# phonchi/Cryo-RAlib

Hardware: AMD Instinct MI355X
Metric: particles/sec aligned, 90x90 nref=10 xr=yr=3 ou=36 (higher is better)
Workload: dtype f32

## Files before the change

cryo_ralib_amd/api.py:

```python
import ctypes
import os

import numpy as np

from ._common import Launcher, ptr

_HERE = os.path.dirname(os.path.abspath(__file__))
LIB_PATH = os.environ.get("RALIGN_LIB") or os.path.join(_HERE, "libralign_hip.so")

RA_MODE_MREF = 0
RA_MODE_REFFREE = 1
RA_INTERP_BILINEAR = 0
RA_INTERP_QUADRI = 1


class AlignConfig(ctypes.Structure):
    _fields_ = [("sbj_num", ctypes.c_uint), ("ref_num", ctypes.c_uint), ("img_dim", ctypes.c_uint),
                ("ring_num", ctypes.c_uint), ("ring_len", ctypes.c_uint),
                ("shift_step", ctypes.c_float), ("shift_rng_x", ctypes.c_float), ("shift_rng_y", ctypes.c_float)]


class AlignParam(ctypes.Structure):
    _fields_ = [("sbj_id", ctypes.c_int), ("ref_id", ctypes.c_int), ("shift_x", ctypes.c_float),
                ("shift_y", ctypes.c_float), ("angle", ctypes.c_float), ("mirror", ctypes.c_bool)]
# ... 21 lines not shown


class RaLdsRow(ctypes.Structure):
    _fields_ = [("kernel", ctypes.c_char * 64), ("static_bytes", ctypes.c_int), ("dynamic_bytes", ctypes.c_int),
                ("limit_bytes", ctypes.c_int)]


float_ptr = ctypes.POINTER(ctypes.c_float)
aln_param_ptr = ctypes.POINTER(AlignParam)

EXPORTED_SYMBOLS = [
    "print_gpu_info", "gpu_clear", "pre_align_init", "pre_align_size_check", "pre_align_fetch",
    "pre_align_run", "pre_align_run_m", "mref_align_run", "mref_align_run_m", "get_num_ref", "reset_shifts",
    "ref_free_alignment_2D_init", "ref_free_alignment_2D_size_check", "ref_free_alignment_2D",
    "ref_free_alignment_2D_filter_references", "ra_isac_get_references", "ra_legacy_bytes",
    "ra_last_error", "ra_create", "ra_destroy", "ra_set_stream", "ra_num_shifts", "ra_maxrin", "ra_lcirc", "ra_search_path", "ra_search_tiled", "ra_search_offsets_per_pass", "ra_set_nomirror", "ra_set_mask",
    "ra_reset_shifts", "ra_set_references", "ra_get_prepared_references", "ra_align", "ra_state_from_params", "ra_set_refine", "ra_set_class_references", "ra_align_classes",
    "ra_debug_spectra", "ra_transform_accumulate", "ra_update_references", "ra_normalize_particles", "ra_sync", "ra_kernel_time",
    "ra_fsc_len", "ra_class_fsc", "ra_last_class_fsc", "ra_fit_tanh", "ra_class_averages", "ra_filter_references",
    "ra_state_from_params_dev", "ra_class_fsc_fit", "ra_filter_references_dev", "ra_last_refine_count", "ra_lds_report",
    "ra_create_ex", "ra_set_normalize_ring", "ra_get_options", "ra_search_skips_offsets", "ra_phase_flip",
    "ra_sdr_mean", "ra_sdr_gram", "ra_sdr_project", "ra_sdr_factors", "ra_rot_shift2d", "ra_sdr_reconstruct",
    "ra_tsne_knn", "ra_tsne_affinity", "ra_tsne_step", "ra_tsne_error",
    "ra_tsne_knn_query", "ra_tsne_affinity_rows", "ra_tsne_place_gradient", "ra_tsne_place",
    "ra_kmeans_sqnorm", "ra_kmeans_labels", "ra_kmeans_lloyd", "ra_kmeans_search", "ra_kmeans_seed",
    "ra_kmeans_silhouette", "ra_kmeans_dispersion", "ra_gmm_estep", "ra_gmm_mstep", "ra_dbscan_count", "ra_dbscan_step",
    "ra_hdbscan_core", "ra_hdbscan_round", "ra_ward_nearest", "ra_ward_merge", "ra_embed_ranks",
    "ra_spectral_spmv", "ra_spectral_lanczos", "ra_spectral_ritz", "ra_spectral_components", "ra_spectral_work_bytes",
    "ra_umap_smooth_knn", "ra_umap_epochs", "ra_umap_place",
    "ra_fourier_resize", "ra_wiener_accumulate", "ra_wiener_finalize", "ra_wiener_frc", "ra_wiener_finalize_ssnr", "ra_wiener_score",
    "ra_prep_normalize", "ra_prep_filter",
# ... 17 lines not shown
    L = ctypes.CDLL(p)
    vp = ctypes.c_void_p
    L.ra_last_error.restype = ctypes.c_char_p
    L.ra_create.argtypes = [ctypes.POINTER(vp), ctypes.POINTER(RaConfig)]
    L.ra_create_ex.argtypes = [ctypes.POINTER(vp), ctypes.POINTER(RaConfig), ctypes.POINTER(RaOptions)]
    L.ra_set_normalize_ring.argtypes = [vp, ctypes.c_int]
    L.ra_get_options.argtypes = [vp, ctypes.POINTER(RaOptions)]
    L.ra_destroy.argtypes = [vp]
    L.ra_destroy.restype = None
    L.ra_set_stream.argtypes = [vp, vp]
    L.ra_num_shifts.argtypes = [vp]
    L.ra_maxrin.argtypes = [vp]
    L.ra_lcirc.argtypes = [vp]
    L.ra_search_path.argtypes = [vp]
    L.ra_search_tiled.argtypes = [vp]
    L.ra_search_skips_offsets.argtypes = [vp]
    L.ra_search_offsets_per_pass.argtypes = [vp]
    L.ra_set_nomirror.argtypes = [vp, ctypes.c_int]
    L.ra_set_mask.argtypes = [vp, vp]
    L.ra_reset_shifts.argtypes = [vp, ctypes.c_float, ctypes.c_float, ctypes.c_float]
    L.ra_set_references.argtypes = [vp, vp]
    L.ra_get_prepared_references.argtypes = [vp, vp]
    L.ra_align.argtypes = [vp, vp, ctypes.c_int, vp, vp, float_ptr]
    L.ra_set_class_references.argtypes = [vp, vp, ctypes.c_int]
    L.ra_align_classes.argtypes = [vp, vp, ctypes.c_int, vp, vp, vp]
    L.ra_state_from_params.argtypes = [vp, vp, ctypes.c_int, float_ptr, vp]
    L.ra_set_refine.argtypes = [vp, ctypes.c_float]
    L.ra_last_refine_count.argtypes = [vp]
    L.ra_lds_report.argtypes = [vp, ctypes.POINTER(RaLdsRow), ctypes.c_int]
    L.ra_state_from_params_dev.argtypes = [vp, vp, ctypes.c_int, vp, vp]
# ... 497 lines not shown
    def align(self, particles, state, result, cs=None):
        n = particles.shape[0]
        assert particles.shape[1:] == (self.nx, self.nx) and state.shape == (n, 2) and result.shape == (n, 8)
        csp = None
        if cs is not None:
            csp = (ctypes.c_float * 2)(float(cs[0]), float(cs[1]))
        _check(self.lib.ra_align(self.handle, self._ptr(particles, self.torch.float32), n,
                                 self._ptr(state, self.torch.float32), self._ptr(result, self.torch.int32), csp),
               "ra_align")

    @property
    def search_tiled(self):
        return bool(self.lib.ra_search_tiled(self.handle))

    @property
    def search_skips_offsets(self):
        return bool(self.lib.ra_search_skips_offsets(self.handle))

    @property
    def search_offsets_per_pass(self):
        return self.lib.ra_search_offsets_per_pass(self.handle)

    def set_refine(self, threshold):
        _check(self.lib.ra_set_refine(self.handle, float(threshold)), "ra_set_refine")

    def state_from_params(self, result, state, cs=None):
        n = result.shape[0]
        assert state.shape == (n, 2) and result.shape == (n, 8)
        csp = None
        if cs is not None:
# ... 115 lines not shown
```

cryo_ralib_amd/csrc/ralign_engine.hip:

```cpp
#include <hip/hip_runtime.h>

#include <algorithm>
#include <cmath>
#include <cstdio>
#include <cstdlib>
#include <cstring>
#include <string>
#include <vector>

#include "ralign_geom.h"
#include "ralign_kernels.h"
#include "ralign_generic.h"
#include "ralign_xform.h"
#include "ralign_zone.h"
#include "ralign_fused.h"
#include "ralign_tiled.h"
#include "ralign_solo.h"
#include "ralign_duo.h"
#include "ralign_pair.h"
#include "ralign_exact.h"
#include "ralign_refine.h"
#include "ralign_host.h"
#include "ralign_plan.h"

// ... 228 lines not shown
    case 128: R1 = 16; R2 = 8; return true;
    case 256: R1 = 16; R2 = 16; return true;
    default: return false;
    }
}

typedef void (*gpolar_fn)(DevGeom, const float *, const float *, int, float *, float2 *);
static gpolar_fn gpolar_kernel(const ra_engine *e, bool refs)
{
    const bool q = e->dg.interp == RA_INTERP_QUADRI;
    return refs ? (q ? (gpolar_fn)polar_generic_kernel<true, true> : (gpolar_fn)polar_generic_kernel<true, false>)
                : (q ? (gpolar_fn)polar_generic_kernel<false, true> : (gpolar_fn)polar_generic_kernel<false, false>);
}

static fused_fn select_tiled(int nh, int sbuf);
static fused_fn select_fused(int maxrin, int nref, int nzr, int sbuf, bool pack = false, bool crop = false);
static bool tcrop_wanted(ra_engine *e, const PlanRequest &rq)
{
    const Geometry &g = e->geo;
    if (!tcrop_class(g, e->cfg, rq, e->generic)) return false;
    FusedGeom t{};
    crop_plan(g, t, rq.sw.crop);
    if (!t.s_crop) return false;
    const int sbuf = (g.lring + 31) / 32 * 32 + 16;
    FusedPlanHost tmp;
    const int pst_min = t.s_pst;
    for (int pst : {pst_min < 101 && !(RA_EXP_ENV("RALIGN_CROP_PST101") && ra_atoi(RA_EXP_ENV("RALIGN_CROP_PST101")) == 0) ? 101 : pst_min, pst_min}) {
    e->crop_pst = pst;
    const size_t polar = (size_t)pst * pst + 4 * (size_t)std::max(sbuf, sbuf <= RF_SBUF_FIXED ? RF_SBUF_FIXED : sbuf) + 2 * g.maxrin + 3000;
    const bool no_tiled = rq.sw.tiled == 0;
    for (int sb : {sbuf <= RF_SBUF_FIXED ? RF_SBUF_FIXED : sbuf, sbuf}) {
// ... 384 lines not shown
}

extern "C" const char *ra_last_error(void) { return g_last_error.c_str(); }

static ccf_fn select_ccf(int maxrin)
{
    switch (maxrin) {
    case 256: return ccf_kernel<256>;
    case 128: return ccf_kernel<128>;
    case 64: return ccf_kernel<64>;
    case 32: return ccf_kernel<32>;
    default: return nullptr;
    }
}

static fused_fn select_fused(int maxrin, int nref, int nzr, int sbuf, bool pack, bool crop)
{
    if (nref > RF_MAXREF) return nullptr;
    const int nrp = (nref + 1) / 2;
    const bool one = nzr == 1;
    if (crop) {
        if (maxrin != 256 || (pack && !one)) return nullptr;
        switch ((nrp + 1) / 2) {
        case 1: return pack ? search_fused_kernel<256, 1, true, 0, true, true> : one ? search_fused_kernel<256, 1, true, 0, false, true> : search_fused_kernel<256, 1, false, 0, false, true>;
        case 2: return pack ? search_fused_kernel<256, 2, true, 0, true, true> : one ? search_fused_kernel<256, 2, true, 0, false, true> : search_fused_kernel<256, 2, false, 0, false, true>;
        case 3: return pack ? search_fused_kernel<256, 3, true, 0, true, true> : one ? search_fused_kernel<256, 3, true, 0, false, true> : search_fused_kernel<256, 3, false, 0, false, true>;
        default: return pack ? search_fused_kernel<256, 4, true, 0, true, true> : one ? search_fused_kernel<256, 4, true, 0, false, true> : search_fused_kernel<256, 4, false, 0, false, true>;
        }
    }
    if (pack) {
        if (maxrin != 256 || !one) return nullptr;
        if (sbuf == RF_SBUF_FIXED)
            switch ((nrp + 1) / 2) {
            case 1: return search_fused_kernel<256, 1, true, RF_SBUF_FIXED, true>;
            case 2: return search_fused_kernel<256, 2, true, RF_SBUF_FIXED, true>;
// ... 84 lines not shown
    const bool no_tiled = rq.sw.tiled == 0;
    auto plan_tiled = [&]() { return build_tiled_plan(g, e->cfg.nref, e->dg.sbuf, e->lds_polar / sizeof(float), fp) && select_tiled(fp.f.nh, e->dg.sbuf); };
    auto plan_fused = [&]() { return select_fused(g.maxrin, e->cfg.nref, 1, 0, false, e->tcrop) && build_fused_plan(g, e->cfg.nref, e->dg.sbuf, e->lds_polar / sizeof(float), fp); };
    if (e->want.tiled && plan_tiled()) e->tiled = true;
    else if (plan_fused()) e->tiled = false;
    else if (e->tcrop && !no_tiled && plan_tiled()) e->tiled = true;
    else if (e->tcrop) {
        g_last_error = "particle-resident search over a crop: the plan tcrop_wanted promised does not fit";
        return RA_ERR_STATE;
    } else return RA_OK;
    if (e->tcrop) {
        FusedGeom tcr{};
        crop_plan(g, tcr, rq.sw.crop);
        fp.f.s_crop = tcr.s_crop; fp.f.s_cropm = tcr.s_cropm;
    }
    int rc;
    if ((rc = upload_resident_tables(e))) return rc;
    for (int pk = 0; pk < (e->tiled ? 1 : 2); pk++) {
        const fused_fn fk = e->tiled ? select_tiled(fp.f.nh, e->dg.sbuf) : select_fused(g.maxrin, e->cfg.nref, fp.f.nzr, e->dg.sbuf, pk != 0, e->tcrop);
        (pk ? e->search.pack : e->search.fused) = fk;
        if (!fk) continue;
        const std::string kn = std::string(e->tiled ? "search_tiled_kernel" : pk ? "search_fused_kernel<pack>" : "search_fused_kernel") + (e->tcrop ? " (crop)" : "");
        if ((rc = raise_dynamic_lds(e, (const void *)fk, kn.c_str(), fp.lds_bytes))) return rc;
    }
    e->search.lds = fp.lds_bytes;
    if (rq.sw.info) fprintf(stderr, "libralign_hip: %s plan: %zu bytes of LDS (polar part %zu), sbuf %d, pst %d, nzr %d, rz %d\n", e->tiled ? "tiled" : "fused", fp.lds_bytes, e->lds_polar, e->dg.sbuf, e->dg.pst, fp.f.nzr, fp.f.rz);
    e->fused = true;
    return RA_OK;
}

static solo_fn select_solo(int maxrin, int nh, int ntile)
{
    if (maxrin != 512) return nullptr;
    if (ntile > 1)
// ... 468 lines not shown
    if (hipStreamSynchronize(e->stream) != hipSuccess || hipMemcpy(&h, e->d_rcount, sizeof(int), hipMemcpyDeviceToHost) != hipSuccess) return RA_ERR_HIP;
    return h;
}
extern "C" int ra_lds_report(const ra_engine *e, ra_lds_row *rows, int cap)
{
    if (!e || cap < 0 || (cap > 0 && !rows)) return RA_ERR_ARG;
    const int n = (int)e->lds_rows.size();
    for (int i = 0; i < std::min(n, cap); i++) {
        const LdsRow &r = e->lds_rows[i];
        snprintf(rows[i].kernel, sizeof(rows[i].kernel), "%s", r.kernel.c_str());
        rows[i].static_bytes = r.stat; rows[i].dynamic_bytes = r.dyn; rows[i].limit_bytes = r.limit;
    }
    return n;
}
extern "C" int ra_search_tiled(const ra_engine *e) { return !e ? RA_ERR_ARG : (e->fused && e->tiled) ? 1 : 0; }
extern "C" int ra_search_path(const ra_engine *e) { return !e ? RA_ERR_ARG : e->solo ? 3 : e->fused ? 1 : e->generic ? 2 : 0; }
extern "C" int ra_search_offsets_per_pass(const ra_engine *e) { return !e ? RA_ERR_ARG : !e->solo ? 0 : (e->duo || e->pair) ? 2 : 1; }
extern "C" int ra_search_skips_offsets(const ra_engine *e) { return !e ? RA_ERR_ARG : (e->solo || e->dg.ent_base) ? 1 : 0; }
extern "C" int ra_num_shifts(const ra_engine *e) { return e ? e->geo.nshift : RA_ERR_ARG; }
extern "C" int ra_maxrin(const ra_engine *e) { return e ? e->geo.maxrin : RA_ERR_ARG; }
extern "C" int ra_lcirc(const ra_engine *e) { return e ? e->geo.lcirc : RA_ERR_ARG; }

extern "C" int ra_reset_shifts(ra_engine *e, float xrng, float yrng, float step)
{
    if (!e) return RA_ERR_ARG;
    const PlanRequest rq{read_switches(), e->force_generic, false, false};
    Geometry g2 = e->geo;
    if (!build_shifts(g2, xrng, yrng, step)) { g_last_error = "bad shift window"; return RA_ERR_ARG; }
    if (g2.nshift_pad > e->pad_cap || g2.nshift > e->shift_cap) {
        g_last_error = "reset_shifts: more search offsets than the engine was created with";
// ... 866 lines not shown
```

cryo_ralib_amd/csrc/ralign_fused.h:

```cpp
#pragma once

#include <algorithm>
#include <cstdlib>
#include <vector>

#include "ralign_geom.h"
#include "ralign_kernels.h"

namespace ralign {

constexpr int RF_WAVES = 16;
constexpr int RF_THREADS = RF_WAVES * 64;
constexpr int RF_MAXREF = 16;

struct FusedGeom {
    int on;
    int ng;
    int wpg;
    int nrp;
    int nrpw;
    int rz, nzr, rz_inv;
    int b_floats;
    int grp_ring0[16];
    int s_crop, s_cropm;
// ... 10 lines not shown
    int ntile, nh;
    int ifft_full;
    int s_pst, s_rows;
    int s_sbuf;
    int s_rank[16];
    int s_call[16];
    int s_stat, s_ctr, s_rec;
    int s_r2;
};

struct FusedPlanHost {
    FusedGeom f{};
    std::vector<int> bsrc;
    std::vector<float> cdc_w;
    size_t lds_bytes = 0;
};

inline int rf_bsrc_code(const Geometry &g, int k, int r, int ref, int part)
{
    if (r >= g.nring) return -1;
    const int n = g.numr[3 * r + 2];
    int ks = k;
    if (k == 0 && part == 1) {
        if (n != g.maxrin) return -1;
        ks = n / 2; part = 0;
    } else if (k > n / 2 || (k == n / 2 && n == g.maxrin)) return -1;
    else if (k == n / 2 && part == 1) return -1;
    const int e = g.bin_off[ks] + (r - g.bin_first[ks]);
    return (e << 8) | (ref << 1) | part;
}
// ... 242 lines not shown
    {
        if (!on) return;
#ifdef RALIGN_PROFILE_SWITCHES
        if (tl && threadIdx.x % 64 == 0) tl[13] = clock64();
#endif
        while (__builtin_amdgcn_readfirstlane(__hip_atomic_load(done, __ATOMIC_RELAXED, __HIP_MEMORY_SCOPE_WORKGROUP)) < target)
            __builtin_amdgcn_s_sleep(1);
        __builtin_amdgcn_fence(__ATOMIC_ACQUIRE, "workgroup", "local");
#ifdef RALIGN_PROFILE_SWITCHES
        if (tl && threadIdx.x % 64 == 0) tl[14] = clock64();
#endif
    }
};

#define RF_SBUF_FIXED 6432
template <int N, int NRPW, bool ONE, int SB, bool PACK = false, bool CROP = false>
__global__ __launch_bounds__(RF_THREADS) void search_fused_kernel(DevGeom g_in, FusedGeom f, const float *__restrict__ particles,
                                                                  const float *__restrict__ state, int n,
                                                                  const float *__restrict__ Bf0, int nref,
                                                                  CandT *__restrict__ cand, const int *__restrict__ cls)
{
    DevGeom g = g_in;
    g.maxrin = N; g.lg_maxrin = __builtin_ctz(N);
    if constexpr (SB != 0) g.sbuf = SB;
    constexpr int R1 = IfftPlan<N>::R1, R2 = IfftPlan<N>::R2;
    extern __shared__ __align__(16) float lds[];
    const int npad = g.pst * g.pst;
    float *img = lds;
    float *bufs = lds + ((npad + 3) & ~3);
    float2 *tw_s = reinterpret_cast<float2 *>(bufs + 4 * g.sbuf);
    float2 *qt_s = tw_s + g.maxrin;
    int4 *inst_s = reinterpret_cast<int4 *>(qt_s + g.n_qtab + (g.n_qtab & 1));
    int4 *jobs_s = inst_s + g.n_inst;
    float *instw_s = reinterpret_cast<float *>(jobs_s + g.n_job);
    float *red = instw_s + g.n_inst;
    float2 *tws = reinterpret_cast<float2 *>(red + 24 + 8 * g.nring + ((g.n_inst + 8 * g.nring) & 1));
// ... 59 lines not shown
            float *dst = img + (y + g.bd) * g.pst + g.bd;
#pragma unroll 1
            for (int c0 = 0; c0 < g.nx; c0 += 64)
                if (c0 + lane < g.nx)
                    __builtin_amdgcn_global_load_lds(row + c0 + lane, (__attribute__((address_space(3))) void *)(dst + c0), 4, 0, 0);
        }
        asm volatile("s_waitcnt vmcnt(0)" ::: "memory");
    };
    auto write_centre = [&](int i0, int s0, int k) {
        int i = i0, sk = s0 + k;
        if (sk >= SPP) { sk -= SPP; i++; }
        i = min(i, npw - 1);
        const int pk = particle_of(i);
        const Window wk = particle_window(g, state[2 * pk], state[2 * pk + 1]);
        const int si = min(sk, g.nshift - 1);
        red[16 + 2 * k] = ((float)g.cnx + wk.sxi) + g.shift_x[si];
        red[17 + 2 * k] = ((float)g.cnx + wk.syi) + g.shift_y[si];
        red[7] = 0.f;
    };
    if (tid < 4 && npw > 0) write_centre(0, 0, (int)tid);
    RF_LDS_BARRIER();
    const int4 jd0 = jobs_s[min((int)wave, g.n_job - 1)];
    constexpr bool defer = ONE;
    auto reduce_records = [&](int i0r, int s0r, int nl) {
        constexpr int W = sizeof(CandT) / 4;
        if (wave == 2 && lane < nl * W) {
            const int o = lane / W, wd = lane - o * W;
            float bv = pc[o * nref].val, sv = -3.0e38f; int br = 0, sr = 0;
            for (int q3 = 1; q3 < nref; q3++) {
                const float v = pc[o * nref + q3].val;
                if (v >= bv) { sv = bv; sr = br; bv = v; br = q3; }
                else if (v >= sv) { sv = v; sr = q3; }
// ... 16 lines not shown
        const int a = min(4, SPP - s0);
        const bool split = PACK && a < nlive;
        const float *Bf = cls ? Bf0 + (size_t)cls[particle_of(i0)] * f.b_floats : Bf0;
        const bool pend = defer && grp > 0;
        if (!RA_DBG(g, 16)) {
#pragma unroll 1
            for (int ph = 0; ph < (split ? 2 : 1); ph++) {
                if (img_i != i0 + ph) {
                    if (ph) RF_LDS_BARRIER();
                    load_image(i0 + ph);
                    img_i = i0 + ph;
                    RF_LDS_BARRIER();
                }
                const int slo = ph ? a : 0, shi = (split && !ph) ? a : nlive;
                const bool wait = pend && !ph;
#pragma unroll 1
                for (int jr = 0; jr * RF_WAVES < g.n_job; jr++) {
                    const int job = jr * RF_WAVES + wave;
                    if (job >= g.n_job) continue;
                    const int4 jd = jr == 0 ? jd0 : jobs_s[job];
#ifdef RALIGN_PROFILE_SWITCHES
                    const PassSync ps = {wait && jr == 0, ifft_done, done_target, g.timeline && tl && grp < 64 ? g.timeline + (grp * 16 + wave) * 16 : nullptr};
#else
                    const PassSync ps = {wait && jr == 0, ifft_done, done_target};
#endif
                    switch (__builtin_amdgcn_readfirstlane(jd.x)) {
                    case 1: ring_job<8, 8, true, true>(g, imgb, bufs, tw_s, qt_s, red + 16, red + 24, inst_s, instw_s, jd.y, jd.z, jd.w, g.sbuf, shi, ps, slo); break;
                    case 6: ring_job<16, 8, true, true>(g, imgb, bufs, tw_s, qt_s, red + 16, red + 24, inst_s, instw_s, jd.y, jd.z, jd.w, g.sbuf, shi, ps, slo); break;
                    case 7: ring_job<8, 4, true, true>(g, imgb, bufs, tw_s, qt_s, red + 16, red + 24, inst_s, instw_s, jd.y, jd.z, jd.w, g.sbuf, shi, ps, slo); break;
                    case 9: ring_job_mix<true>(g, imgb, bufs, tw_s, qt_s, red + 16, red + 24, inst_s, instw_s, jd.y, jd.z, jd.w, g.sbuf, shi, ps, slo); break;
                    default: break;
                    }
                }
                if (wait && wave >= g.n_job) { const PassSync ps = {true, ifft_done, done_target}; ps(); }
            }
        } else if (pend) {
            const PassSync ps = {true, ifft_done, done_target};
            ps();
        }
        if (pend) reduce_records(i0p, s0p, nlp);
        RA_STAMP(g, tl, grp, wave, 1);
        const int ln = __builtin_amdgcn_mbcnt_hi(~0u, __builtin_amdgcn_mbcnt_lo(~0u, __float_as_int(red[7])));
        float4 b0[NRPW];
        {
            const float *bp = Bf + f.grp_boff[xm] + ln * 4;
// ... 148 lines not shown
```

cryo_ralib_amd/csrc/ralign_kernels.h:

```cpp
#pragma once

#include <hip/hip_runtime.h>
#include <stdint.h>

#include "ralign_fft.h"
#include "../../include/ralign.h"

#ifdef RALIGN_PROFILE_SWITCHES
#define RA_DBG(g, bits) (((g).dbg & (bits)) != 0)
#define RA_STAMP(g, cond, grp, wave, s)                                                                         \
    do { if ((g).timeline && (cond) && (grp) < 64 && threadIdx.x % 64 == 0) (g).timeline[((grp) * 16 + (wave)) * 16 + (s)] = clock64(); } while (0)
#else
#define RA_DBG(g, bits) false
#define RA_STAMP(g, cond, grp, wave, s) do { } while (0)
#endif

namespace ralign {

typedef float f32x4 __attribute__((ext_vector_type(4)));

struct DevGeom {
    int nx, cnx;
    int nring, maxrin, lcirc, lring, nbins, LB, LBP;
    int last_ring;
// ... 137 lines not shown
    int idx;
    asm("v_mad_i32_i24 %0, %1, %2, %3" : "=v"(idx) : "v"(iy), "s"(st), "v"(ix));
    const float *p = base + idx;
#ifdef RALIGN_BILINEAR_EXACT_ORDER
    const float f00 = p[0], f10 = p[1], f01 = p[st], f11 = p[st + 1];
    return f00 + ydif * (f01 - f00) + xdif * (f10 - f00 + ydif * (f11 - f10 - f01 + f00));
#else
    const v2f r0 = {p[0], p[1]}, r1 = {p[st], p[st + 1]};
    const v2f g = __builtin_elementwise_fma((v2f){ydif, ydif}, r1 - r0, r0);
    float d = g.y - g.x;
    asm("" : "+v"(d));
    return __builtin_fmaf(xdif, d, g.x);
#endif
}

struct Window { float sxi, syi; int lkx, rkx, lky, rky; };
__device__ __forceinline__ Window particle_window(const DevGeom &g, float dx, float dy)
{
    Window w;
    const float mashi = (float)(g.cnx - g.win_ring - 2);
    if (g.mode == RA_MODE_MREF) {
        if (fabsf(dx) > mashi || fabsf(dy) > mashi) { dx = 0.f; dy = 0.f; }
    } else {
        dx = fminf(fmaxf(dx, -mashi), mashi);
        dy = fminf(fmaxf(dy, -mashi), mashi);
    }
    w.sxi = dx; w.syi = dy;
    const int cn = g.nx / 2 + 1;
    float qlx = fmaxf(cn + dx - g.win_ring - 2, 0.f), qex = fmaxf(g.nx - cn - dx - g.win_ring, 0.f);
    float qly = fmaxf(cn + dy - g.win_ring - 2, 0.f), qey = fmaxf(g.nx - cn - dy - g.win_ring, 0.f);
// ... 141 lines not shown
    do {                                                             \
        __builtin_amdgcn_fence(__ATOMIC_RELEASE, "workgroup");       \
        asm volatile("s_waitcnt lgkmcnt(0)" ::: "memory");           \
        __builtin_amdgcn_wave_barrier();                             \
        __builtin_amdgcn_fence(__ATOMIC_ACQUIRE, "workgroup");       \
    } while (0)

#ifdef RALIGN_MARK_PHASES
#define RA_PHASE_MARK(name) asm volatile("; RA_PHASE " name)
#else
#define RA_PHASE_MARK(name) do {} while (0)
#endif

struct NoSync { __device__ __forceinline__ void operator()() const {} };

template <int R1, int LR, bool NYQ1 = false, bool EARLY = false, class Sync = NoSync>
__device__ __forceinline__ void ring_job(const DevGeom &g, const float *imgb, float *bufs, const float2 *tw_s,
                                         const float2 *qt_s, const float *ctr, float *part, const int4 *inst_s,
                                         const float *instw_s, int inst0, int count, int zero, int sbuf, int nlive = 4,
                                         Sync sync = Sync(), int slot_lo = 0)
{
    const int lane = __builtin_amdgcn_mbcnt_hi(~0u, __builtin_amdgcn_mbcnt_lo(~0u, zero));

    constexpr int H = R1 * LR, NR = 2 * H, LT = NR / 4;
    const int sub = lane / LR, t = lane % LR;
    const int subc = min(sub, count - 1);
    const int4 in = inst_s[inst0 + subc];
    const int slot = in.x & 255, ring = in.x >> 8;
    const bool active = sub < count && slot < nlive && slot >= slot_lo;
    float *buf = bufs + (__mul24(slot, sbuf) + in.y);
    const float rad = (float)in.w, wt = instw_s[inst0 + subc];
    const float cx = ctr[2 * slot], cy = ctr[2 * slot + 1];
    const float2 *qt = qt_s + in.z;
    v2f av2 = {0.f, 0.f}, sq2 = {0.f, 0.f};
    const v2f ctr2 = {cx, cy};
    float2 v[R1];
    constexpr bool QCT = (2 * LR <= LT) && (R1 >= 4);
    constexpr int NB = QCT ? R1 / 4 : R1;
    auto table_index = [&](int step, int u, int &qd) {
        if constexpr (QCT) { qd = 0; return 2 * LR * step + 2 * t + u; }
        else { const int j = 2 * (LR * step + t) + u; qd = j / LT; return j % LT; }
    };
    if (active) {
    int qdn[2];
    float2 scn[2];
#pragma unroll
    for (int u = 0; u < 2; u++) scn[u] = qt[table_index(0, u, qdn[u])];
#pragma unroll
// ... 14 lines not shown
        for (int q = 0; q < (QCT ? 4 : 1); q++) {
            const int a = QCT ? q * NB + b : b;
            v2f val;
#pragma unroll
            for (int u = 0; u < 2; u++) {
                v2f o;
                if constexpr (QCT) {
                    o = q == 0 ? ctr2 + xy[u] : q == 1 ? vadd_rot<-1>(ctr2, xy[u]) : q == 2 ? ctr2 - xy[u] : vadd_rot<1>(ctr2, xy[u]);
                } else {
                    const int qd = qdc[u];
                    v2f m = (qd & 1) ? v2f{xy[u].y, xy[u].x} : xy[u];
                    m.x = (qd & 2) ? -m.x : m.x;
                    m.y = ((qd + 1) & 2) ? -m.y : m.y;
                    o = m + ctr2;
                }
                const float s = bilinear_pad(imgb, g.pst, o.x, o.y);
                if (u == 0) val.x = s; else val.y = s;
            }
            av2 += val;
            sq2 += val * val;
            v[a] = make_float2(val.x, val.y);
            if ((NYQ1 && (QCT ? 4 * b + q : b) >= R1 / 2) || ((QCT ? q : b) & 1)) __builtin_amdgcn_sched_barrier(0);
        }
    }
    }
    sync();
    if (!active) return;
    float av = (av2.x + av2.y) * wt, sq = (sq2.x + sq2.y) * wt;
    if (RA_DBG(g, 256)) {
#pragma unroll
        for (int a = 0; a < R1; a++) *reinterpret_cast<float2 *>(buf + 2 * (LR * a + t)) = v[a];
        return;
    }
    RA_PHASE_MARK("ring_fft_begin");
    Dft<-1, R1>::run(v);
    constexpr int LGH = __builtin_ctz(H), LGNR = LGH + 1;
    const int tstep = t << (g.lg_maxrin - LGH);
// ... 106 lines not shown
                } else {
                    float2 zm = *reinterpret_cast<const float2 *>(buf + 2 * (H - k));
                    v2f xk, xm;
                    vsplit_pair(to_v(zk), to_v(zm), to_v(tw_s[k << lsh]), xk, xm);
                    *reinterpret_cast<float2 *>(buf + 2 * k) = to_f2(xk);
                    if (2 * k != H) *reinterpret_cast<float2 *>(buf + 2 * (H - k)) = to_f2(xm);
                }
            }
        }
    }
    RA_PHASE_MARK("ring_fft_end");
    av = group_sum_dpp<LR>(av); sq = group_sum_dpp<LR>(sq);
    if (t == 0) { part[2 * (slot * g.nring + ring)] = av; part[2 * (slot * g.nring + ring) + 1] = sq; }
}

template <bool NYQ1, class Sync = NoSync>
__device__ __forceinline__ void ring_job_mix(const DevGeom &g, const float *imgb, float *bufs, const float2 *tw_s,
                                             const float2 *qt_s, const float *ctr, float *part, const int4 *inst_s,
                                             const float *instw_s, int inst0, int count, int zero, int sbuf, int nlive = 4,
                                             Sync sync = Sync(), int slot_lo = 0)
{
    const int lane = __builtin_amdgcn_mbcnt_hi(~0u, __builtin_amdgcn_mbcnt_lo(~0u, zero));
    const int lanec = min(lane, count - 1);
    const int4 in = inst_s[inst0 + lanec];
    const int slot = in.x & 255, ring = (in.x >> 8) & 255, lg = (in.x >> 16) & 15, t = in.x >> 20;
    const bool active = lane < count && slot < nlive && slot >= slot_lo;
    const int lgLR = lg - 3, LR = 1 << lgLR, H = 4 << lgLR, lgLT = lg - 2, LTm = (1 << lgLT) - 1;
    float *buf = bufs + (__mul24(slot, sbuf) + in.y);
    const float rad = (float)in.w, wt = instw_s[inst0 + lanec];
    const v2f ctr2 = {ctr[2 * slot], ctr[2 * slot + 1]};
    const float2 *qt = qt_s + in.z;
    v2f av2 = {0.f, 0.f}, sq2 = {0.f, 0.f};
    float2 v[4];
    if (active) {
#pragma unroll
    for (int a = 0; a < 4; a++) {
        v2f val;
#pragma unroll
        for (int u = 0; u < 2; u++) {
            const int j = 2 * ((a << lgLR) + t) + u, qd = j >> lgLT;
            const float2 sc = qt[j & LTm];
            v2f o;
            {
#pragma clang fp contract(off)
                const v2f xy = v2f{sc.x, sc.y} * rad;
                v2f m = (qd & 1) ? v2f{xy.y, xy.x} : xy;
                m.x = (qd & 2) ? -m.x : m.x;
                m.y = ((qd + 1) & 2) ? -m.y : m.y;
                o = m + ctr2;
            }
            const float sv = bilinear_pad(imgb, g.pst, o.x, o.y);
            if (u == 0) val.x = sv; else val.y = sv;
        }
        av2 += val;
        sq2 += val * val;
        v[a] = make_float2(val.x, val.y);
    }
    }
    sync();
    if (!active) return;
    Dft<-1, 4>::run(v);
    const int tstep = t << (g.lg_maxrin - (lg - 1));
#pragma unroll
    for (int c = 0; c < 4; c++) {
        float2 o = v[c];
        if (c > 0) o = cmul(o, tw_s[__mul24(tstep, c)]);
// ... 947 lines not shown
```

cryo_ralib_amd/csrc/ralign_plan.h:

```cpp
#pragma once

#include <cstdlib>

#include "../../include/ralign.h"
#include "ralign_geom.h"
#include "ralign_fused.h"
#include "ralign_tiled.h"
#include "ralign_solo.h"
#include "ralign_pair.h"

namespace ralign {

inline int env_int(const char *name, int unset) { const char *v = getenv(name); return v ? atoi(v) : unset; }
inline bool env_set(const char *name) { return getenv(name) != nullptr; }

struct PlanSwitches {
    bool generic, fused, solo, pair, duo, tcrop, crop, tight_rings, zones, live_offsets, gccf_split, refine_gm, atomic_sums, info;
    int tiled;
    int gccf_tm;
    int solo_jobs;
    int grid;
    const char *refine;
};
inline PlanSwitches read_switches()
// ... 48 lines not shown
}
inline bool duo_class(const Geometry &g, const ra_config &cfg, const PlanRequest &rq, bool generic)
{
    return solo_class(g, cfg, rq, generic) && rq.sw.duo;
}
inline bool pair_class(const Geometry &g, const ra_config &cfg, const PlanRequest &rq, bool generic)
{
    return generic && g.maxrin == 256 && g.nring <= 4 * RP_NQ && g.numr[2] >= 8 && cfg.nref <= 127 && !rq.generic_forced() && rq.sw.pair;
}
inline bool tcrop_class(const Geometry &g, const ra_config &cfg, const PlanRequest &rq, bool generic)
{
    return generic && g.maxrin == 256 && g.nring <= 64 && g.numr[2] >= 8 && cfg.nref <= 127 && !rq.generic_forced() &&
           rq.allow_tcrop && rq.sw.tcrop && rq.sw.fused;
}

inline size_t b_stream_quads(const Geometry &g)
{
    size_t quads = 0;
    for (int m = 0; m < g.maxrin / 32; m++) {
        int r0 = 0;
        while (r0 < g.nring) {
            const int n = g.numr[3 * r0 + 2], nbin = (n == g.maxrin) ? n / 2 : n / 2 + 1;
            if (16 * m < nbin) break;
            r0++;
        }
        quads += (g.nring - r0 + 3) / 4;
    }
    return quads;
}

// ... 2 lines not shown
```

include/ralign.h:

```cpp
#ifndef RALIGN_H
#define RALIGN_H

#include <stdbool.h>
#include <stddef.h>

#ifdef __cplusplus
extern "C" {
#endif


typedef struct AlignConfig {
    unsigned int sbj_num;
    unsigned int ref_num;
    unsigned int img_dim;
    unsigned int ring_num;
    unsigned int ring_len;
    float shift_step;
    float shift_rng_x;
    float shift_rng_y;
} AlignConfig;

typedef struct AlignParam {
    int   sbj_id;
    int   ref_id;
// ... 69 lines not shown

const char *ra_last_error(void);
int  ra_create(ra_engine **out, const ra_config *cfg);
int  ra_create_ex(ra_engine **out, const ra_config *cfg, const ra_options *opt);
int  ra_set_normalize_ring(ra_engine *e, int flag);
int  ra_get_options(const ra_engine *e, ra_options *opt);
void ra_destroy(ra_engine *e);
int  ra_set_stream(ra_engine *e, void *hip_stream);
int  ra_num_shifts(const ra_engine *e);
int  ra_maxrin(const ra_engine *e);
int  ra_lcirc(const ra_engine *e);
int  ra_search_path(const ra_engine *e);
int  ra_search_offsets_per_pass(const ra_engine *e);
int  ra_search_skips_offsets(const ra_engine *e);
int  ra_search_tiled(const ra_engine *e);
int  ra_reset_shifts(ra_engine *e, float xrng, float yrng, float step);

int  ra_set_mask(ra_engine *e, const float *d_mask);

int  ra_set_nomirror(ra_engine *e, int flag);

int  ra_set_references(ra_engine *e, const float *d_refs);
int  ra_get_prepared_references(ra_engine *e, float *h_crefim);

int  ra_align(ra_engine *e, const float *d_particles, int n, float *d_state,
              ra_result *d_result, const float *cs);
int  ra_set_refine(ra_engine *e, float threshold);
int  ra_last_refine_count(ra_engine *e);
typedef struct ra_lds_row {
    char kernel[64];
// ... 142 lines not shown
```

Baseline: 1.695 million.

## Sample inner polar rings directly from global memory through L1 instead of LDS

For the fused 256-sample search kernel, rings with up to 64 or 128 samples now read their bilinear taps straight from the particle image in global memory (through the L1 cache) rather than from the padded LDS copy. A planner rule checks that every such ring, at every shift, stays inside the image, and clamps shift centres so the unpadded reads cannot go out of bounds. New template instantiations, scheduling barriers and query entry points are added. The aim is to take load off LDS bandwidth and capacity, with the risk of higher global-load latency and more kernel variants.

```diff
diff --git a/cryo_ralib_amd/api.py b/cryo_ralib_amd/api.py
--- a/cryo_ralib_amd/api.py
+++ b/cryo_ralib_amd/api.py
@@ -59,7 +59,7 @@
     "pre_align_run", "pre_align_run_m", "mref_align_run", "mref_align_run_m", "get_num_ref", "reset_shifts",
     "ref_free_alignment_2D_init", "ref_free_alignment_2D_size_check", "ref_free_alignment_2D",
     "ref_free_alignment_2D_filter_references", "ra_isac_get_references", "ra_legacy_bytes",
-    "ra_last_error", "ra_create", "ra_destroy", "ra_set_stream", "ra_num_shifts", "ra_maxrin", "ra_lcirc", "ra_search_path", "ra_search_tiled", "ra_search_offsets_per_pass", "ra_set_nomirror", "ra_set_mask",
+    "ra_last_error", "ra_create", "ra_destroy", "ra_set_stream", "ra_num_shifts", "ra_maxrin", "ra_lcirc", "ra_search_path", "ra_search_tiled", "ra_search_l1_tap_rings", "ra_l1_tap_rule", "ra_search_offsets_per_pass", "ra_set_nomirror", "ra_set_mask",
     "ra_reset_shifts", "ra_set_references", "ra_get_prepared_references", "ra_align", "ra_state_from_params", "ra_set_refine", "ra_set_class_references", "ra_align_classes",
     "ra_debug_spectra", "ra_transform_accumulate", "ra_update_references", "ra_normalize_particles", "ra_sync", "ra_kernel_time",
     "ra_fsc_len", "ra_class_fsc", "ra_last_class_fsc", "ra_fit_tanh", "ra_class_averages", "ra_filter_references",
@@ -107,6 +107,9 @@
     L.ra_lcirc.argtypes = [vp]
     L.ra_search_path.argtypes = [vp]
     L.ra_search_tiled.argtypes = [vp]
+    if hasattr(L, "ra_search_l1_tap_rings"):
+        L.ra_search_l1_tap_rings.argtypes = [vp]
+        L.ra_l1_tap_rule.argtypes = [ctypes.c_int] * 4 + [ctypes.c_float] * 2
     L.ra_search_skips_offsets.argtypes = [vp]
     L.ra_search_offsets_per_pass.argtypes = [vp]
     L.ra_set_nomirror.argtypes = [vp, ctypes.c_int]
@@ -634,6 +637,10 @@
         return bool(self.lib.ra_search_tiled(self.handle))
 
     @property
+    def search_l1_tap_rings(self):
+        return self.lib.ra_search_l1_tap_rings(self.handle)
+
+    @property
     def search_skips_offsets(self):
         return bool(self.lib.ra_search_skips_offsets(self.handle))
 
diff --git a/cryo_ralib_amd/csrc/ralign_engine.hip b/cryo_ralib_amd/csrc/ralign_engine.hip
--- a/cryo_ralib_amd/csrc/ralign_engine.hip
+++ b/cryo_ralib_amd/csrc/ralign_engine.hip
@@ -266,7 +266,7 @@
 }
 
 static fused_fn select_tiled(int nh, int sbuf);
-static fused_fn select_fused(int maxrin, int nref, int nzr, int sbuf, bool pack = false, bool crop = false);
+static fused_fn select_fused(int maxrin, int nref, int nzr, int sbuf, bool pack = false, bool crop = false, int tapl1 = 0);
 static bool tcrop_wanted(ra_engine *e, const PlanRequest &rq)
 {
     const Geometry &g = e->geo;
@@ -681,11 +681,26 @@
     }
 }
 
-static fused_fn select_fused(int maxrin, int nref, int nzr, int sbuf, bool pack, bool crop)
+static bool fused_tap_family(int maxrin, int nzr, int sbuf, bool crop) { return maxrin == 256 && nzr == 1 && sbuf == RF_SBUF_FIXED && !crop; }
+template <int TAPL1> static fused_fn select_fused_tap(int nrp, bool pack)
+{
+    switch ((nrp + 1) / 2) {
+    case 1: return pack ? search_fused_kernel<256, 1, true, RF_SBUF_FIXED, true, false, TAPL1> : search_fused_kernel<256, 1, true, RF_SBUF_FIXED, false, false, TAPL1>;
+    case 2: return pack ? search_fused_kernel<256, 2, true, RF_SBUF_FIXED, true, false, TAPL1> : search_fused_kernel<256, 2, true, RF_SBUF_FIXED, false, false, TAPL1>;
+    case 3: return pack ? search_fused_kernel<256, 3, true, RF_SBUF_FIXED, true, false, TAPL1> : search_fused_kernel<256, 3, true, RF_SBUF_FIXED, false, false, TAPL1>;
+    default: return nullptr;
+    }
+}
+
+static fused_fn select_fused(int maxrin, int nref, int nzr, int sbuf, bool pack, bool crop, int tapl1)
 {
     if (nref > RF_MAXREF) return nullptr;
     const int nrp = (nref + 1) / 2;
     const bool one = nzr == 1;
+    if (tapl1) {
+        if (!fused_tap_family(maxrin, nzr, sbuf, crop)) return nullptr;
+        return tapl1 == 128 ? select_fused_tap<128>(nrp, pack) : tapl1 == 64 ? select_fused_tap<64>(nrp, pack) : nullptr;
+    }
     if (crop) {
         if (maxrin != 256 || (pack && !one)) return nullptr;
         switch ((nrp + 1) / 2) {
@@ -800,10 +815,14 @@
         crop_plan(g, tcr, rq.sw.crop);
         fp.f.s_crop = tcr.s_crop; fp.f.s_cropm = tcr.s_cropm;
     }
+    fp.tap_l1 = 0;
+    const int tap_cap = (e->dg.dbg & 16384) ? 0 : RA_EXP_ENV("RALIGN_TAPL1") ? ra_atoi(RA_EXP_ENV("RALIGN_TAPL1")) : kTapL1Cap;
+    if (!e->tiled && fused_tap_family(g.maxrin, fp.f.nzr, e->dg.sbuf, e->tcrop) && fp.f.nrp >= 2 && fp.f.nrp <= 5)
+        fp.tap_l1 = l1_tap_rings(g.numr, g.nring, g.nx, g.last_ring, e->cfg.xrng, e->cfg.yrng, std::min(tap_cap, kTapL1Cap));
     int rc;
     if ((rc = upload_resident_tables(e))) return rc;
     for (int pk = 0; pk < (e->tiled ? 1 : 2); pk++) {
-        const fused_fn fk = e->tiled ? select_tiled(fp.f.nh, e->dg.sbuf) : select_fused(g.maxrin, e->cfg.nref, fp.f.nzr, e->dg.sbuf, pk != 0, e->tcrop);
+        const fused_fn fk = e->tiled ? select_tiled(fp.f.nh, e->dg.sbuf) : select_fused(g.maxrin, e->cfg.nref, fp.f.nzr, e->dg.sbuf, pk != 0, e->tcrop, fp.tap_l1);
         (pk ? e->search.pack : e->search.fused) = fk;
         if (!fk) continue;
         const std::string kn = std::string(e->tiled ? "search_tiled_kernel" : pk ? "search_fused_kernel<pack>" : "search_fused_kernel") + (e->tcrop ? " (crop)" : "");
@@ -1302,6 +1321,16 @@
     return n;
 }
 extern "C" int ra_search_tiled(const ra_engine *e) { return !e ? RA_ERR_ARG : (e->fused && e->tiled) ? 1 : 0; }
+extern "C" int ra_l1_tap_rule(int nx, int first_ring, int last_ring, int ring_skip, float xrng, float yrng)
+{
+    Geometry g;
+    if (nx < 1 || !build_rings(g, nx, first_ring, last_ring, ring_skip > 0 ? ring_skip : 1) || xrng < 0.f || yrng < 0.f) {
+        g_last_error = "bad ring or window arguments";
+        return RA_ERR_ARG;
+    }
+    return l1_tap_rings(g.numr, g.nring, nx, last_ring, xrng, yrng);
+}
+extern "C" int ra_search_l1_tap_rings(const ra_engine *e) { return !e ? RA_ERR_ARG : (e->fused && !e->tiled) ? e->fplan.tap_l1 : 0; }
 extern "C" int ra_search_path(const ra_engine *e) { return !e ? RA_ERR_ARG : e->solo ? 3 : e->fused ? 1 : e->generic ? 2 : 0; }
 extern "C" int ra_search_offsets_per_pass(const ra_engine *e) { return !e ? RA_ERR_ARG : !e->solo ? 0 : (e->duo || e->pair) ? 2 : 1; }
 extern "C" int ra_search_skips_offsets(const ra_engine *e) { return !e ? RA_ERR_ARG : (e->solo || e->dg.ent_base) ? 1 : 0; }
diff --git a/cryo_ralib_amd/csrc/ralign_fused.h b/cryo_ralib_amd/csrc/ralign_fused.h
--- a/cryo_ralib_amd/csrc/ralign_fused.h
+++ b/cryo_ralib_amd/csrc/ralign_fused.h
@@ -48,6 +48,7 @@
     std::vector<int> bsrc;
     std::vector<float> cdc_w;
     size_t lds_bytes = 0;
+    int tap_l1 = 0;
 };
 
 inline int rf_bsrc_code(const Geometry &g, int k, int r, int ref, int part)
@@ -320,12 +321,13 @@
 };
 
 #define RF_SBUF_FIXED 6432
-template <int N, int NRPW, bool ONE, int SB, bool PACK = false, bool CROP = false>
+template <int N, int NRPW, bool ONE, int SB, bool PACK = false, bool CROP = false, int TAPL1 = 0>
 __global__ __launch_bounds__(RF_THREADS) void search_fused_kernel(DevGeom g_in, FusedGeom f, const float *__restrict__ particles,
                                                                   const float *__restrict__ state, int n,
                                                                   const float *__restrict__ Bf0, int nref,
                                                                   CandT *__restrict__ cand, const int *__restrict__ cls)
 {
+    static_assert(TAPL1 == 0 || (!CROP && (TAPL1 == 64 || TAPL1 == 128)), "taps through the L1: whole-image kernels, rings up to 64 or 128 samples");
     DevGeom g = g_in;
     g.maxrin = N; g.lg_maxrin = __builtin_ctz(N);
     if constexpr (SB != 0) g.sbuf = SB;
@@ -415,8 +417,15 @@
         const int pk = particle_of(i);
         const Window wk = particle_window(g, state[2 * pk], state[2 * pk + 1]);
         const int si = min(sk, g.nshift - 1);
-        red[16 + 2 * k] = ((float)g.cnx + wk.sxi) + g.shift_x[si];
-        red[17 + 2 * k] = ((float)g.cnx + wk.syi) + g.shift_y[si];
+        float cx = ((float)g.cnx + wk.sxi) + g.shift_x[si], cy = ((float)g.cnx + wk.syi) + g.shift_y[si];
+        if constexpr (TAPL1 > 0) {
+            const int mashi = abs(g.cnx - g.win_ring - 2);
+            const float mx = (float)(mashi + (int)ceilf(g.xrng)), my = (float)(mashi + (int)ceilf(g.yrng));
+            cx = fminf(fmaxf(cx, (float)g.cnx - mx), (float)g.cnx + mx);
+            cy = fminf(fmaxf(cy, (float)g.cnx - my), (float)g.cnx + my);
+        }
+        red[16 + 2 * k] = cx;
+        red[17 + 2 * k] = cy;
         red[7] = 0.f;
     };
     if (tid < 4 && npw > 0) write_centre(0, 0, (int)tid);
@@ -463,6 +472,10 @@
                 }
                 const int slo = ph ? a : 0, shi = (split && !ph) ? a : nlive;
                 const bool wait = pend && !ph;
+                constexpr int T128 = TAPL1 >= 128 ? TAP_L1 : TAP_LDS, T64 = TAPL1 >= 64 ? TAP_L1 : TAP_LDS;
+                const float *gimg = imgb;
+                if constexpr (TAPL1 > 0) gimg = particles + ((long long)particle_of(i0 + ph) * (g.nx * g.nx) - (g.nx + 1));
+                const float *tap128 = T128 == TAP_L1 ? gimg : imgb, *tap64 = T64 == TAP_L1 ? gimg : imgb;
 #pragma unroll 1
                 for (int jr = 0; jr * RF_WAVES < g.n_job; jr++) {
                     const int job = jr * RF_WAVES + wave;
@@ -474,10 +487,10 @@
                     const PassSync ps = {wait && jr == 0, ifft_done, done_target};
 #endif
                     switch (__builtin_amdgcn_readfirstlane(jd.x)) {
-                    case 1: ring_job<8, 8, true, true>(g, imgb, bufs, tw_s, qt_s, red + 16, red + 24, inst_s, instw_s, jd.y, jd.z, jd.w, g.sbuf, shi, ps, slo); break;
+                    case 1: ring_job<8, 8, true, true, T128>(g, tap128, bufs, tw_s, qt_s, red + 16, red + 24, inst_s, instw_s, jd.y, jd.z, jd.w, g.sbuf, shi, ps, slo); break;
                     case 6: ring_job<16, 8, true, true>(g, imgb, bufs, tw_s, qt_s, red + 16, red + 24, inst_s, instw_s, jd.y, jd.z, jd.w, g.sbuf, shi, ps, slo); break;
-                    case 7: ring_job<8, 4, true, true>(g, imgb, bufs, tw_s, qt_s, red + 16, red + 24, inst_s, instw_s, jd.y, jd.z, jd.w, g.sbuf, shi, ps, slo); break;
-                    case 9: ring_job_mix<true>(g, imgb, bufs, tw_s, qt_s, red + 16, red + 24, inst_s, instw_s, jd.y, jd.z, jd.w, g.sbuf, shi, ps, slo); break;
+                    case 7: ring_job<8, 4, true, true, T64>(g, tap64, bufs, tw_s, qt_s, red + 16, red + 24, inst_s, instw_s, jd.y, jd.z, jd.w, g.sbuf, shi, ps, slo); break;
+                    case 9: ring_job_mix<true, T64>(g, tap64, bufs, tw_s, qt_s, red + 16, red + 24, inst_s, instw_s, jd.y, jd.z, jd.w, g.sbuf, shi, ps, slo); break;
                     default: break;
                     }
                 }
diff --git a/cryo_ralib_amd/csrc/ralign_kernels.h b/cryo_ralib_amd/csrc/ralign_kernels.h
--- a/cryo_ralib_amd/csrc/ralign_kernels.h
+++ b/cryo_ralib_amd/csrc/ralign_kernels.h
@@ -175,6 +175,54 @@
 #endif
 }
 
+enum { TAP_LDS = 0, TAP_L1 = 1 };
+typedef float v2f_a4 __attribute__((ext_vector_type(2), aligned(4)));
+
+__device__ __forceinline__ float bilinear_l1(const float *base, int nx, float xold, float yold)
+{
+#pragma clang fp contract(off)
+    const int ix = (int)xold, iy = (int)yold;
+    const float ydif = __builtin_amdgcn_fractf(yold), xdif = __builtin_amdgcn_fractf(xold);
+    int idx;
+    asm("v_mad_i32_i24 %0, %1, %2, %3" : "=v"(idx) : "v"(iy), "s"(nx), "v"(ix));
+    const char *b = reinterpret_cast<const char *>(base);
+    const unsigned o0 = 4u * (unsigned)idx, o1 = o0 + 4u * (unsigned)nx;
+    const v2f r0 = *reinterpret_cast<const v2f_a4 *>(b + o0), r1 = *reinterpret_cast<const v2f_a4 *>(b + o1);
+    const v2f g = __builtin_elementwise_fma((v2f){ydif, ydif}, r1 - r0, r0);
+    float d = g.y - g.x;
+    asm("" : "+v"(d));
+    return __builtin_fmaf(xdif, d, g.x);
+}
+
+#ifdef RALIGN_PROFILE_SWITCHES
+__device__ __forceinline__ float bilinear_probe(const float *base, int st, float xold, float yold, int lane)
+{
+#pragma clang fp contract(off)
+    const int ix = (int)xold, iy = (int)yold;
+    const float ydif = __builtin_amdgcn_fractf(yold), xdif = __builtin_amdgcn_fractf(xold);
+    int idx;
+    asm volatile("v_mad_i32_i24 %0, %1, %2, %3" : "=v"(idx) : "v"(iy), "s"(st), "v"(ix));
+    const float *p = base + lane;
+    const v2f r0 = {p[0], p[1]}, r1 = {p[st], p[st + 1]};
+    const v2f g = __builtin_elementwise_fma((v2f){ydif, ydif}, r1 - r0, r0);
+    float d = g.y - g.x;
+    asm("" : "+v"(d));
+    return __builtin_fmaf(xdif, d, g.x);
+}
+#endif
+
+template <int TAP>
+__device__ __forceinline__ float ring_tap_sample(const DevGeom &g, const float *imgb, float x, float y, bool probe, int lane)
+{
+    if constexpr (TAP == TAP_L1) return bilinear_l1(imgb, g.nx, x, y);
+    else {
+#ifdef RALIGN_PROFILE_SWITCHES
+        if (probe) return bilinear_probe(imgb, g.pst, x, y, lane);
+#endif
+        return bilinear_pad(imgb, g.pst, x, y);
+    }
+}
+
 struct Window { float sxi, syi; int lkx, rkx, lky, rky; };
 __device__ __forceinline__ Window particle_window(const DevGeom &g, float dx, float dy)
 {
@@ -346,7 +394,7 @@
 
 struct NoSync { __device__ __forceinline__ void operator()() const {} };
 
-template <int R1, int LR, bool NYQ1 = false, bool EARLY = false, class Sync = NoSync>
+template <int R1, int LR, bool NYQ1 = false, bool EARLY = false, int TAP = TAP_LDS, class Sync = NoSync>
 __device__ __forceinline__ void ring_job(const DevGeom &g, const float *imgb, float *bufs, const float2 *tw_s,
                                          const float2 *qt_s, const float *ctr, float *part, const int4 *inst_s,
                                          const float *instw_s, int inst0, int count, int zero, int sbuf, int nlive = 4,
@@ -364,6 +412,7 @@
     const float rad = (float)in.w, wt = instw_s[inst0 + subc];
     const float cx = ctr[2 * slot], cy = ctr[2 * slot + 1];
     const float2 *qt = qt_s + in.z;
+    const bool probe = NR <= 128 && RA_DBG(g, 16384);
     v2f av2 = {0.f, 0.f}, sq2 = {0.f, 0.f};
     const v2f ctr2 = {cx, cy};
     float2 v[R1];
@@ -408,13 +457,15 @@
                     m.y = ((qd + 1) & 2) ? -m.y : m.y;
                     o = m + ctr2;
                 }
-                const float s = bilinear_pad(imgb, g.pst, o.x, o.y);
+                const float s = ring_tap_sample<TAP>(g, imgb, o.x, o.y, probe, lane);
                 if (u == 0) val.x = s; else val.y = s;
             }
             av2 += val;
             sq2 += val * val;
             v[a] = make_float2(val.x, val.y);
-            if ((NYQ1 && (QCT ? 4 * b + q : b) >= R1 / 2) || ((QCT ? q : b) & 1)) __builtin_amdgcn_sched_barrier(0);
+            if constexpr (TAP == TAP_L1) {
+                if (QCT ? q == 3 : (b & 3) == 3) __builtin_amdgcn_sched_barrier(0);
+            } else if ((NYQ1 && (QCT ? 4 * b + q : b) >= R1 / 2) || ((QCT ? q : b) & 1)) __builtin_amdgcn_sched_barrier(0);
         }
     }
     }
@@ -551,7 +602,7 @@
     if (t == 0) { part[2 * (slot * g.nring + ring)] = av; part[2 * (slot * g.nring + ring) + 1] = sq; }
 }
 
-template <bool NYQ1, class Sync = NoSync>
+template <bool NYQ1, int TAP = TAP_LDS, class Sync = NoSync>
 __device__ __forceinline__ void ring_job_mix(const DevGeom &g, const float *imgb, float *bufs, const float2 *tw_s,
                                              const float2 *qt_s, const float *ctr, float *part, const int4 *inst_s,
                                              const float *instw_s, int inst0, int count, int zero, int sbuf, int nlive = 4,
@@ -567,6 +618,7 @@
     const float rad = (float)in.w, wt = instw_s[inst0 + lanec];
     const v2f ctr2 = {ctr[2 * slot], ctr[2 * slot + 1]};
     const float2 *qt = qt_s + in.z;
+    const bool probe = RA_DBG(g, 16384);
     v2f av2 = {0.f, 0.f}, sq2 = {0.f, 0.f};
     float2 v[4];
     if (active) {
@@ -586,7 +638,7 @@
                 m.y = ((qd + 1) & 2) ? -m.y : m.y;
                 o = m + ctr2;
             }
-            const float sv = bilinear_pad(imgb, g.pst, o.x, o.y);
+            const float sv = ring_tap_sample<TAP>(g, imgb, o.x, o.y, probe, lane);
             if (u == 0) val.x = sv; else val.y = sv;
         }
         av2 += val;
diff --git a/cryo_ralib_amd/csrc/ralign_plan.h b/cryo_ralib_amd/csrc/ralign_plan.h
--- a/cryo_ralib_amd/csrc/ralign_plan.h
+++ b/cryo_ralib_amd/csrc/ralign_plan.h
@@ -1,6 +1,9 @@
 #pragma once
 
+#include <algorithm>
+#include <cmath>
 #include <cstdlib>
+#include <vector>
 
 #include "../../include/ralign.h"
 #include "ralign_geom.h"
@@ -86,6 +89,30 @@
            rq.allow_tcrop && rq.sw.tcrop && rq.sw.fused;
 }
 
+constexpr int kTapL1Cap = 128;
+inline int l1_tap_mashi(const std::vector<int> &numr, int nring, int nx, int last_ring)
+{
+    const int cn = nx / 2 + 1;
+    return std::max(std::abs(cn - last_ring - 2), std::abs(cn - numr[3 * (nring - 1)] - 2));
+}
+inline bool l1_tap_ring_ok(int nx, int mashi, float xrng, float yrng, int r)
+{
+    const int cn = nx / 2 + 1, ax = mashi + (int)std::ceil(xrng), ay = mashi + (int)std::ceil(yrng);
+    return cn - ax - r >= 1 && cn + ax + r + 1 <= nx && cn - ay - r >= 1 && cn + ay + r + 1 <= nx;
+}
+inline int l1_tap_rings(const std::vector<int> &numr, int nring, int nx, int last_ring, float xrng, float yrng, int cap = kTapL1Cap)
+{
+    const int mashi = l1_tap_mashi(numr, nring, nx, last_ring);
+    for (int T : {128, 64}) {
+        if (T > cap) continue;
+        bool ok = true;
+        for (int i = 0; i < nring && ok; i++)
+            if (numr[3 * i + 2] <= T && !l1_tap_ring_ok(nx, mashi, xrng, yrng, numr[3 * i])) ok = false;
+        if (ok) return T;
+    }
+    return 0;
+}
+
 inline size_t b_stream_quads(const Geometry &g)
 {
     size_t quads = 0;
diff --git a/include/ralign.h b/include/ralign.h
--- a/include/ralign.h
+++ b/include/ralign.h
@@ -107,6 +107,8 @@
 int  ra_search_offsets_per_pass(const ra_engine *e);
 int  ra_search_skips_offsets(const ra_engine *e);
 int  ra_search_tiled(const ra_engine *e);
+int  ra_search_l1_tap_rings(const ra_engine *e);
+int  ra_l1_tap_rule(int nx, int first_ring, int last_ring, int ring_skip, float xrng, float yrng);
 int  ra_reset_shifts(ra_engine *e, float xrng, float yrng, float step);
 
 int  ra_set_mask(ra_engine *e, const float *d_mask);
```

Result: faster. 1.716 million, median of 6 (+1.3%).
